# liamliaw/medical-image-segmentation-with-visual-prompts

Hardware: NVIDIA B200
Metric: 3D patches/sec fwd+bwd (96^3 SwinUNETR+prompts) at 1/2/4/8 B200; attn TFLOP/s (higher is better)
Workload: dtype bf16

## Files before the change

### include/pwa.h

```cpp
#ifndef PWA_H_
#define PWA_H_

#include <stddef.h>
#include <stdint.h>

#ifdef __cplusplus
extern "C" {
#endif

#define PWA_VERSION 100

enum { PWA_OK = 0, PWA_ERR_ARG = -1, PWA_ERR_UNSUPPORTED = -2, PWA_ERR_CUDA = -3 };
enum { PWA_F32 = 0, PWA_BF16 = 1 };

typedef struct pwa_geom {
  int32_t dims[3];
  int32_t ws[3];
  int32_t shift[3];
  int32_t pads[6];
  int32_t sp[3];
  int32_t nwin[3];
  int32_t data_lo[3];
  int32_t crop_lo[3];
  int32_t P;
  int32_t N;
  int32_t masked;
  int32_t padded;
} pwa_geom;


int pwa_version(void);
const char* pwa_last_error(void);

int pwa_geometry(const int32_t dims[3], const int32_t ws[3], const int32_t shift_cfg[3], pwa_geom* out);

int pwa_region_ids(const pwa_geom* g, uint8_t* ids_host);

int pwa_attn_sel_table(const uint8_t* ids_host, int P, int N, uint32_t* table_host);

int pwa_index_map(const pwa_geom* g, int which, int32_t* map_host);


int pwa_partition(const void* x, void* tokens, int B, int C, const pwa_geom* g, int use_crop_lo,
                  int dtype, void* stream);

int pwa_reverse(const void* tokens, void* x, int B, int C, const pwa_geom* g, int use_crop_lo,
                int dtype, void* stream);

int pwa_reverse_add(const void* tokens_a, const void* tokens_b, void* x, int B, int C, const pwa_geom* g,
                    int use_crop_lo, int dtype, void* stream);

int pwa_gather_rows(const void* src_a, const void* src_b, void* dst, const int32_t* map, int B,
                    int64_t rows_src, int64_t rows_dst, int C, int dtype, void* stream);

int pwa_colsum_f32(const float* src, float* dst, int S, int64_t n, void* stream);

int pwa_colsum_rows(const void* x, float* dst, int64_t rows, int C, int dtype, void* stream);

int pwa_dropout(const void* x, void* y, int64_t n, float p_drop, const void* seed_dev, int dtype, void* stream);

int pwa_dropout_colsum(const void* x, void* y, int64_t rows, int C, float p_drop, const void* seed_dev, float* colsum,
                       int dtype, void* stream);


typedef struct pwa_attn_shape {
  int32_t B, P, C, heads, I;
  int32_t ws[3];
  float scale;
  float p_drop;
  uint64_t seed, offset;
  int32_t ld_qkv;
  int32_t ld_p;
  const void* seed_dev;
  const void* sel_table;
  void* work;
} pwa_attn_shape;

int pwa_attn_fwd(const void* q, const void* k, const void* v, const void* kp, const void* vp,
                 const float* th, const float* tw, const float* td, const float* tok,
                 const uint8_t* ids, void* out, float* lse, const pwa_attn_shape* s, int dtype,
                 int impl, void* stream);


int pwa_attn_bwd(const void* q, const void* k, const void* v, const void* kp, const void* vp,
                 const float* th, const float* tw, const float* td, const float* tok,
                 const uint8_t* ids, const void* out, const float* lse, const void* dout,
                 void* dq, void* dk, void* dv, float* dkp, float* dvp,
                 float* dth, float* dtw, float* dtd, float* dtok, float* delta,
                 const pwa_attn_shape* s, int dtype, int impl, void* stream);


int pwa_bias_tables_fwd(const float* enc_h, const float* enc_w, const float* enc_d, const float* wc_h,
                        const float* wc_w, const float* wc_d, const float* enc_tok, const float* w_tok,
                        float* th, float* tw, float* td, float* tok, int heads, int E, const int32_t ws[3],
                        const int32_t cap[3], int I, void* stream);

int pwa_bias_tables_bwd(const float* enc_h, const float* enc_w, const float* enc_d, const float* wc_h,
                        const float* wc_w, const float* wc_d, const float* enc_tok, const float* w_tok,
                        const float* dth, const float* dtw, const float* dtd, const float* dtok,
                        float* denc_h, float* denc_w, float* denc_d, float* dwc_h, float* dwc_w, float* dwc_d,
                        float* denc_tok, float* dw_tok, int heads, int E, const int32_t ws[3],
                        const int32_t cap[3], int I, void* stream);


int pwa_ln_fwd(const void* x, const void* res, const float* gamma, const float* beta, void* sum_out, void* y,
               float* mean, float* rstd, int64_t rows, int C, float eps, int dtype, void* stream);

int pwa_ln_bwd(const void* dy, const void* x, const float* gamma, const float* mean, const float* rstd,
               const void* dres, void* dx, float* dgamma, float* dbeta, int64_t rows, int C, int dtype, void* stream);

int pwa_ln_bwd2(const void* dy, const void* x, const float* gamma, const float* mean, const float* rstd,
                const void* dres, void* dx, float* dgamma, float* dbeta, float* dres_colsum, float* dx_colsum,
                int64_t rows, int C, int dtype, void* stream);


int pwa_token_gemm_supported(int C, int Cout);
int pwa_token_gemm_fwd(const void* x, const void* res, const float* gamma, const float* beta, const void* W, const void* bias,
                       void* sum_out, void* ln_out, void* y, float* mean, float* rstd, int64_t T, int C, int Cout, float eps,
                       float p_drop, const void* seed_dev, void* stream);

int pwa_attn_tc_supported(const pwa_attn_shape* s, int dtype);

typedef struct pwa_dense_attn {
  int32_t B, P, heads, dh, nq, nk;
  int32_t ld_q, ld_k, ld_v;
  int64_t bias_stride[4];
  int64_t mask_stride[4];
  float scale, p_drop;
  const void* seed_dev;
} pwa_dense_attn;
int pwa_attn_dense_fwd(const void* q, const void* k, const void* v, const float* bias, const float* mask, void* out, float* lse,
                       const pwa_dense_attn* s, int dtype, void* stream);
int pwa_attn_dense_bwd(const void* q, const void* k, const void* v, const float* bias, const float* mask, const void* out,
                       const float* lse, const void* dout, void* dq, void* dk, void* dv, float* dbias, float* delta,
                       const pwa_dense_attn* s, int dtype, void* stream);

#ifdef __cplusplus
}
#endif
#endif
```

### medical-image-segmentation-with-visual-prompts_b200/_lib.py

```python
from __future__ import annotations

import ctypes as C
import os

_HERE = os.path.dirname(os.path.abspath(__file__))
LIB_PATH = os.path.join(_HERE, "libpwa_b200.so")

PWA_F32, PWA_BF16 = 0, 1


class PwaGeom(C.Structure):
    _fields_ = [
        ("dims", C.c_int32 * 3), ("ws", C.c_int32 * 3), ("shift", C.c_int32 * 3), ("pads", C.c_int32 * 6),
        ("sp", C.c_int32 * 3), ("nwin", C.c_int32 * 3), ("data_lo", C.c_int32 * 3), ("crop_lo", C.c_int32 * 3),
        ("P", C.c_int32), ("N", C.c_int32), ("masked", C.c_int32), ("padded", C.c_int32),
    ]


class PwaAttnShape(C.Structure):
    _fields_ = [
        ("B", C.c_int32), ("P", C.c_int32), ("C", C.c_int32), ("heads", C.c_int32), ("I", C.c_int32),
        ("ws", C.c_int32 * 3), ("scale", C.c_float), ("p_drop", C.c_float),
        ("seed", C.c_uint64), ("offset", C.c_uint64), ("ld_qkv", C.c_int32), ("ld_p", C.c_int32),
        ("seed_dev", C.c_void_p), ("sel_table", C.c_void_p), ("work", C.c_void_p),
    ]


class PwaDenseAttn(C.Structure):
    _fields_ = [
        ("B", C.c_int32), ("P", C.c_int32), ("heads", C.c_int32), ("dh", C.c_int32), ("nq", C.c_int32), ("nk", C.c_int32),
        ("ld_q", C.c_int32), ("ld_k", C.c_int32), ("ld_v", C.c_int32),
        ("bias_stride", C.c_int64 * 4), ("mask_stride", C.c_int64 * 4),
        ("scale", C.c_float), ("p_drop", C.c_float), ("seed_dev", C.c_void_p),
    ]


class PwaError(RuntimeError):
    pass


def _load():
    if not os.path.isfile(LIB_PATH):
        raise ImportError(
            f"{LIB_PATH} not found: the CUDA extension is not built. Run "
            "`python -c 'import __graft_entry__ as g; g.build()'` (or `make -C <package>/csrc`). "
            "This package has no CPU or PyTorch fallback.")
    lib = C.CDLL(LIB_PATH)
    vp, i32, f32p, u8p = C.c_void_p, C.c_int32, C.c_void_p, C.c_void_p
    gp, sp = C.POINTER(PwaGeom), C.POINTER(PwaAttnShape)
    lib.pwa_version.restype = i32
    lib.pwa_last_error.restype = C.c_char_p
    lib.pwa_geometry.argtypes = [C.POINTER(i32), C.POINTER(i32), C.POINTER(i32), gp]
    lib.pwa_region_ids.argtypes = [gp, vp]
    lib.pwa_index_map.argtypes = [gp, i32, vp]
    lib.pwa_attn_sel_table.argtypes = [vp, i32, i32, vp]
    lib.pwa_attn_sel_table.restype = i32
    lib.pwa_partition.argtypes = [vp, vp, i32, i32, gp, i32, i32, vp]
    lib.pwa_reverse.argtypes = [vp, vp, i32, i32, gp, i32, i32, vp]
    lib.pwa_reverse_add.argtypes = [vp, vp, vp, i32, i32, gp, i32, i32, vp]
    lib.pwa_reverse_add.restype = i32
    lib.pwa_gather_rows.argtypes = [vp, vp, vp, vp, i32, C.c_int64, C.c_int64, i32, i32, vp]
    lib.pwa_gather_rows.restype = i32
    lib.pwa_colsum_f32.argtypes = [f32p, f32p, i32, C.c_int64, vp]
    lib.pwa_colsum_f32.restype = i32
    lib.pwa_colsum_rows.argtypes = [vp, f32p, C.c_int64, i32, i32, vp]
    lib.pwa_colsum_rows.restype = i32
    lib.pwa_dropout.argtypes = [vp, vp, C.c_int64, C.c_float, vp, i32, vp]
    lib.pwa_dropout.restype = i32
    lib.pwa_dropout_colsum.argtypes = [vp, vp, C.c_int64, i32, C.c_float, vp, vp, i32, vp]
    lib.pwa_dropout_colsum.restype = i32
    lib.pwa_token_gemm_supported.argtypes = [i32, i32]
    lib.pwa_token_gemm_supported.restype = i32
    lib.pwa_token_gemm_fwd.argtypes = [vp] * 11 + [C.c_int64, i32, i32, C.c_float, C.c_float, vp, vp]
    lib.pwa_token_gemm_fwd.restype = i32
    if hasattr(lib, "pwa_debug_fwd_timeline"):
        lib.pwa_debug_fwd_timeline.argtypes = [vp, i32]
        lib.pwa_debug_fwd_timeline.restype = i32
    lib.pwa_attn_tc_supported.argtypes = [sp, i32]
    dp = C.POINTER(PwaDenseAttn)
    lib.pwa_attn_dense_fwd.argtypes = [vp] * 7 + [dp, i32, vp]
    lib.pwa_attn_dense_bwd.argtypes = [vp] * 13 + [dp, i32, vp]
    lib.pwa_attn_dense_fwd.restype = lib.pwa_attn_dense_bwd.restype = i32
    lib.pwa_attn_fwd.argtypes = [vp] * 5 + [f32p] * 4 + [u8p, vp, f32p, sp, i32, i32, vp]
    lib.pwa_attn_bwd.argtypes = [vp] * 5 + [f32p] * 4 + [u8p, vp, f32p, vp] + [vp] * 3 + [f32p] * 7 + [sp, i32, i32, vp]
    i64, f32 = C.c_int64, C.c_float
    lib.pwa_ln_fwd.argtypes = [vp, vp, f32p, f32p, vp, vp, f32p, f32p, i64, i32, f32, i32, vp]
    lib.pwa_ln_bwd.argtypes = [vp, vp, f32p, f32p, f32p, vp, vp, f32p, f32p, i64, i32, i32, vp]
    lib.pwa_ln_bwd2.argtypes = [vp, vp, f32p, f32p, f32p, vp, vp, f32p, f32p, f32p, f32p, i64, i32, i32, vp]
    lib.pwa_ln_fwd.restype = lib.pwa_ln_bwd.restype = lib.pwa_ln_bwd2.restype = i32
    i32p = C.POINTER(i32)
    lib.pwa_bias_tables_fwd.argtypes = [f32p] * 8 + [f32p] * 4 + [i32, i32, i32p, i32p, i32, vp]
    lib.pwa_bias_tables_bwd.argtypes = [f32p] * 8 + [f32p] * 4 + [f32p] * 8 + [i32, i32, i32p, i32p, i32, vp]
    lib.pwa_bias_tables_fwd.restype = lib.pwa_bias_tables_bwd.restype = i32
    for name in ("pwa_geometry", "pwa_region_ids", "pwa_index_map", "pwa_partition", "pwa_reverse",
                 "pwa_attn_tc_supported", "pwa_attn_fwd", "pwa_attn_bwd"):
        getattr(lib, name).restype = i32
    return lib


lib = _load()

EXPORTED_SYMBOLS = ("pwa_version", "pwa_last_error", "pwa_geometry", "pwa_region_ids", "pwa_index_map", "pwa_attn_sel_table",
                    "pwa_partition", "pwa_reverse", "pwa_reverse_add", "pwa_gather_rows", "pwa_colsum_f32", "pwa_colsum_rows", "pwa_dropout", "pwa_dropout_colsum", "pwa_token_gemm_supported", "pwa_token_gemm_fwd", "pwa_attn_fwd", "pwa_attn_bwd", "pwa_attn_tc_supported", "pwa_attn_dense_fwd", "pwa_attn_dense_bwd",
                    "pwa_ln_fwd", "pwa_ln_bwd", "pwa_ln_bwd2", "pwa_bias_tables_fwd", "pwa_bias_tables_bwd")


def check(rc: int, what: str):
    if rc != 0:
        msg = lib.pwa_last_error().decode("utf-8", "replace")
        if rc == -1 and "not compatible with the number of heads" in msg:
            raise ValueError(msg)
        if rc == -2:
            raise NotImplementedError(f"{what}: {msg}")
        raise PwaError(f"{what} failed (rc={rc}): {msg}")
```

### medical-image-segmentation-with-visual-prompts_b200/functional.py

```python
from __future__ import annotations

import ctypes as C
from typing import Optional, Sequence

import functools

import torch

from . import _lib
from .geometry import Geometry

_DT = {torch.float32: _lib.PWA_F32, torch.bfloat16: _lib.PWA_BF16}


class KernelStats:
    enabled = False
    timing = False
    launches = 0
    records = []

    @classmethod
    def reset(cls, enabled=True, timing=False):
        cls.enabled, cls.timing, cls.launches, cls.records = enabled, timing, 0, []

    @classmethod
    def summary(cls):
        out = {}
        for name, e0, e1, work in cls.records:
            c, ms, w = out.get(name, (0, 0.0, 0.0))
            out[name] = (c + 1, ms + e0.elapsed_time(e1), w + work)
        return out


class _timed:
    def __init__(self, name, n_kernels, work, t):
        self.name, self.n, self.work, self.t = name, n_kernels, work, t

    def __enter__(self):
        if KernelStats.enabled:
            KernelStats.launches += self.n
            if KernelStats.timing:
                self.e0 = torch.cuda.Event(enable_timing=True)
                self.e1 = torch.cuda.Event(enable_timing=True)
                self.e0.record(torch.cuda.current_stream(self.t.device))
        return self

    def __exit__(self, *exc):
        if KernelStats.enabled and KernelStats.timing:
            self.e1.record(torch.cuda.current_stream(self.t.device))
            KernelStats.records.append((self.name, self.e0, self.e1, self.work))
        return False


def _dtype_code(t: torch.Tensor) -> int:
    if t.dtype not in _DT:
        raise TypeError(f"pwa kernels support float32 and bfloat16, got {t.dtype}")
    return _DT[t.dtype]


def _require_cuda(*ts):
    for t in ts:
        if t is not None and not t.is_cuda:
            raise RuntimeError("pwa_b200 has no CPU path: tensors must live on a CUDA device (sm_100a)")


def _stream(t: torch.Tensor):
    return C.c_void_p(torch.cuda.current_stream(t.device).cuda_stream)


def _ptr(t: Optional[torch.Tensor]):
    return C.c_void_p(0 if t is None else t.data_ptr())


def _force_bits(force_generic, force_word, force_vec):
    return (2 if force_generic else 0) | (4 if force_word else 0) | (8 if force_vec else 0)


def _partition_raw(x: torch.Tensor, geom: Geometry, crop_lo: int, force_generic: bool = False,
                   force_word: bool = False, force_vec: bool = False) -> torch.Tensor:
    B, Cc = x.shape[:2]
    out = torch.empty((B, geom.P, geom.N, Cc), dtype=x.dtype, device=x.device)
    with torch.cuda.device(x.device), _timed("partition", 1, 2.0 * out.numel() * out.element_size(), x):
        rc = _lib.lib.pwa_partition(_ptr(x), _ptr(out), B, Cc, geom.ref(), crop_lo | _force_bits(force_generic, force_word, force_vec),
                                    _dtype_code(x), _stream(x))
    _lib.check(rc, "pwa_partition")
    return out


def _reverse_raw(tok: torch.Tensor, geom: Geometry, crop_lo: int, force_generic: bool = False,
                 force_word: bool = False, force_vec: bool = False) -> torch.Tensor:
    B, _, _, Cc = tok.shape
    out = torch.empty((B, Cc, *geom.dims), dtype=tok.dtype, device=tok.device)
    with torch.cuda.device(tok.device), _timed("reverse", 1, 2.0 * tok.numel() * tok.element_size(), tok):
        rc = _lib.lib.pwa_reverse(_ptr(tok), _ptr(out), B, Cc, geom.ref(), crop_lo | _force_bits(force_generic, force_word, force_vec),
                                  _dtype_code(tok), _stream(tok))
    _lib.check(rc, "pwa_reverse")
    return out


class _Partition(torch.autograd.Function):
    @staticmethod
    def forward(ctx, x, geom):
        ctx.geom = geom
        return _partition_raw(x.contiguous(), geom, 0)

    @staticmethod
    def backward(ctx, g):
        return _reverse_raw(g.contiguous(), ctx.geom, 0), None


class _Reverse(torch.autograd.Function):
    @staticmethod
    def forward(ctx, tok, geom):
        ctx.geom = geom
        return _reverse_raw(tok.contiguous(), geom, 1)

    @staticmethod
    def backward(ctx, g):
        return _partition_raw(g.contiguous(), ctx.geom, 1), None


class _ReverseAdd(torch.autograd.Function):
    @staticmethod
    def forward(ctx, tok_a, tok_b, geom):
        ctx.geom = geom
        tok_a, tok_b = tok_a.contiguous(), tok_b.contiguous()
        B, _, _, Cc = tok_a.shape
        out = torch.empty((B, Cc, *geom.dims), dtype=tok_a.dtype, device=tok_a.device)
        with torch.cuda.device(tok_a.device), _timed("reverse", 1, 3.0 * tok_a.numel() * tok_a.element_size(), tok_a):
            rc = _lib.lib.pwa_reverse_add(_ptr(tok_a), _ptr(tok_b), _ptr(out), B, Cc, geom.ref(), 1, _dtype_code(tok_a),
                                          _stream(tok_a))
        _lib.check(rc, "pwa_reverse_add")
        return out

    @staticmethod
    def backward(ctx, g):
        d = _partition_raw(g.contiguous(), ctx.geom, 1)
        return d, d, None


def reverse_add_tokens(tok_a: torch.Tensor, tok_b: torch.Tensor, geom: Geometry) -> torch.Tensor:
    _require_cuda(tok_a, tok_b)
    if tok_a.shape != tok_b.shape or tok_a.dtype != tok_b.dtype or tuple(tok_a.shape[1:3]) != (geom.P, geom.N):
        raise ValueError("reverse_add_tokens: mismatching token tensors")
    return _ReverseAdd.apply(tok_a, tok_b, geom)


def partition_tokens(x: torch.Tensor, geom: Geometry) -> torch.Tensor:
    _require_cuda(x)
    if tuple(x.shape[2:]) != geom.dims:
        raise ValueError(f"feature map {tuple(x.shape[2:])} does not match geometry {geom.dims}")
    return _Partition.apply(x, geom)


def reverse_tokens(tok: torch.Tensor, geom: Geometry) -> torch.Tensor:
    _require_cuda(tok)
    if tuple(tok.shape[1:3]) != (geom.P, geom.N):
        raise ValueError(f"token tensor {tuple(tok.shape)} does not match geometry P={geom.P} N={geom.N}")
# ... 511 lines not shown
        return dx, None, None, (None if db is None else db.to(ctx.bias_dtype))


def dropout_colsum_supported(C: int) -> bool:
    return C % 4 == 0 and C <= 1024


def seeded_dropout(x: torch.Tensor, p_drop: float, seed: Optional[torch.Tensor] = None, bias_of_x=None) -> torch.Tensor:
    _require_cuda(x, seed)
    if p_drop <= 0.0:
        return x
    if seed is None:
        seed = new_dropout_seed(x.device)
    if seed.dtype != torch.int32 or seed.numel() < 2:
        raise ValueError("seeded_dropout: seed must be an int32 tensor with two words")
    return _SeededDropout.apply(x, float(p_drop), seed, bias_of_x)


def prompted_window_attention_packed(qkv, kvp, th, tw, td, tok, ids, heads: int, ws: Sequence[int], scale: float,
                                     impl: int = IMPL_AUTO, p_drop: float = 0.0, seed: Optional[torch.Tensor] = None) -> torch.Tensor:
    _require_cuda(qkv, kvp, th, tw, td, tok, ids)
    if qkv.shape[-1] % (3 * heads) != 0:
        raise ValueError('WindowAttention: The dimension is not compatible with the number of heads!')
    if qkv.dim() != 4:
        raise ValueError(f"prompted_window_attention_packed: qkv must be [B,P,N,3C], got {tuple(qkv.shape)}")
    _check_attn_side_inputs(qkv.shape[0], qkv.shape[1], qkv.shape[2], qkv.shape[3] // 3, qkv.dtype, kvp, None, 2, th, tw, td, tok,
                            ids, heads, ws)
    if p_drop > 0 and seed is None:
        seed = new_dropout_seed(qkv.device)
    return _WindowAttentionPacked.apply(qkv, kvp, th, tw, td, tok, ids, heads, tuple(ws), scale, impl, float(p_drop), seed)


def _mm_f32(a, b):
    if a.dtype == torch.float32:
        return torch.mm(a, b)
    try:
        return torch.mm(a, b, out_dtype=torch.float32)
    except (TypeError, RuntimeError):
        return torch.mm(a, b).float()


@functools.lru_cache(maxsize=None)
def _token_split(T):
    cands = [d for d in range(32, 161) if T % d == 0]
    return min(cands, key=lambda d: abs(d - 72)) if cands else 0


def colsum_f32(part):
    _require_cuda(part)
    part = part.contiguous()
    out = torch.empty(part.shape[1:], dtype=torch.float32, device=part.device)
    with torch.cuda.device(part.device), _timed("colsum", 1, 4.0 * part.numel(), part):
        rc = _lib.lib.pwa_colsum_f32(_ptr(part), _ptr(out), part.shape[0], out.numel(), _stream(part))
    _lib.check(rc, "pwa_colsum_f32")
    return out


def colsum_rows(x2):
    _require_cuda(x2)
    T, Cc = x2.shape
    e = 16 // x2.element_size()
    if x2.dtype not in (torch.float32, torch.bfloat16) or not x2.is_contiguous() or Cc % e or Cc // e > 512 or x2.data_ptr() % 16:
        return x2.sum(dim=0, dtype=torch.float32)
    if T == 0:
        return torch.zeros(Cc, dtype=torch.float32, device=x2.device)
    out = torch.empty(Cc, dtype=torch.float32, device=x2.device)
    with torch.cuda.device(x2.device), _timed("colsum_rows", 1, float(x2.numel() * x2.element_size()), x2):
        rc = _lib.lib.pwa_colsum_rows(_ptr(x2), _ptr(out), T, Cc, _dtype_code(x2), _stream(x2))
    _lib.check(rc, "pwa_colsum_rows")
    return out


def _wgrad(dy2, x2):
    T, co = dy2.shape
    ci = x2.shape[1]
    if dy2.dtype != torch.float32 and dy2.is_contiguous() and x2.is_contiguous():
        S = 0
        if T >= 16384 and co * ci <= 40960:
            S = _token_split(T)
        elif T >= 8192 and T % 8 == 0 and co * ci <= 131072:
            S = 8
        if S:
            try:
                part = torch.bmm(dy2.view(S, T // S, co).transpose(1, 2), x2.view(S, T // S, ci), out_dtype=torch.float32)
            except (TypeError, RuntimeError):
                part = None
            if part is not None:
                return colsum_f32(part)
    return _mm_f32(dy2.t(), x2)


class _MultiLinear(torch.autograd.Function):

    @staticmethod
    def forward(ctx, x, bias, lowp, bias_grad, lowp_bias, *weights):
        w = lowp if lowp is not None else (weights[0] if len(weights) == 1 else torch.cat(weights, dim=0)).detach().to(x.dtype)
        x2 = x.reshape(-1, x.shape[-1])
        if bias is not None:
            y = torch.addmm(lowp_bias if lowp_bias is not None else bias.detach().to(x.dtype), x2, w.t())
        else:
            y = torch.mm(x2, w.t())
        ctx.save_for_backward(x2, w)
        ctx.meta = (x.shape, [wt.shape[0] for wt in weights], [wt.dtype for wt in weights],
                    None if (bias is None or not bias_grad) else bias.dtype)
        return y.reshape(*x.shape[:-1], w.shape[0])

    @staticmethod
    def backward(ctx, dy):
        x2, w = ctx.saved_tensors
        xshape, rows, wdts, bdt = ctx.meta
        dy2 = dy.reshape(-1, dy.shape[-1])
        dx = torch.mm(dy2, w).reshape(xshape) if ctx.needs_input_grad[0] else None
        db = colsum_rows(dy2).to(bdt) if bdt is not None and ctx.needs_input_grad[1] else None
        dws = [None] * len(rows)
        if any(ctx.needs_input_grad[5:]):
            dw = _wgrad(dy2, x2)
            o = 0
            for i, r in enumerate(rows):
                if ctx.needs_input_grad[5 + i]:
                    dws[i] = dw[o:o + r].to(wdts[i])
                o += r
        return (dx, db, None, None, None, *dws)


def multi_linear(x, bias, *weights, lowp=None, bias_grad=True, lowp_bias=None):
    return _MultiLinear.apply(x, bias, lowp, bias_grad, lowp_bias, *weights)


def token_gemm_supported(C: int, Cout: int, dtype) -> bool:
    return dtype == torch.bfloat16 and bool(_lib.lib.pwa_token_gemm_supported(int(C), int(Cout)))


def token_gemm_profitable(C: int, rows: int) -> bool:
    return C <= 48 and rows >= 32768


def _token_gemm_raw(x2, res2, g32, b32, w, bias, want_sum, want_ln, want_stats, eps, p_drop, seed):
    rows, Cc = x2.shape
    Cout = w.shape[0]
    dev = x2.device
    y = torch.empty((rows, Cout), dtype=x2.dtype, device=dev)
    s = torch.empty_like(x2) if want_sum else None
    z = torch.empty_like(x2) if want_ln else None
    mean = torch.empty(rows, dtype=torch.float32, device=dev) if want_stats else None
    rstd = torch.empty(rows, dtype=torch.float32, device=dev) if want_stats else None
    nbytes = ((1 if res2 is None else 2) + (1 if want_sum else 0) + (1 if want_ln else 0)) * x2.numel() * 2 + y.numel() * 2
    with torch.cuda.device(dev), _timed("token_gemm", 1, float(nbytes), x2):
        rc = _lib.lib.pwa_token_gemm_fwd(_ptr(x2), _ptr(res2), _ptr(g32), _ptr(b32), _ptr(w), _ptr(bias), _ptr(s), _ptr(z), _ptr(y),
                                         _ptr(mean), _ptr(rstd), rows, Cc, Cout, float(eps), float(p_drop), _ptr(seed), _stream(x2))
    _lib.check(rc, "pwa_token_gemm_fwd")
    return y, s, z, mean, rstd


def _ln_backward_raw(dy, x, g32, mean, rstd, dres, want_res_colsum, want_x_colsum):
    Cc = x.shape[-1]
    rows = x.numel() // Cc
    dx = torch.empty_like(x)
    f32 = dict(dtype=torch.float32, device=x.device)
    dg, db = torch.empty(Cc, **f32), torch.empty(Cc, **f32)
    dbr = torch.empty(Cc, **f32) if want_res_colsum and dres is not None else None
    dbx = torch.empty(Cc, **f32) if want_x_colsum else None
    nbytes = (3 if dres is None else 4) * x.numel() * x.element_size()
    with torch.cuda.device(x.device), _timed("ln_bwd", 1, float(nbytes), x):
        rc = _lib.lib.pwa_ln_bwd2(_ptr(dy), _ptr(x), _ptr(g32), _ptr(mean), _ptr(rstd), _ptr(dres), _ptr(dx), _ptr(dg), _ptr(db),
                                  _ptr(dbr), _ptr(dbx), rows, Cc, _dtype_code(x), _stream(x))
    _lib.check(rc, "pwa_ln_bwd")
    return dx, dg, db, dbr, dbx


class _LnLinearPass(torch.autograd.Function):

    @staticmethod
    def forward(ctx, x, gamma, beta, eps, lowp_w, *weights):
        x = x.contiguous()
        Cc = x.shape[-1]
        g32, b32 = gamma.detach().float().contiguous(), beta.detach().float().contiguous()
        w = lowp_w if lowp_w is not None else (weights[0] if len(weights) == 1 else torch.cat(weights, dim=0)).detach().to(x.dtype)
        w = w.contiguous()
        y, _, tokens, mean, rstd = _token_gemm_raw(x.view(-1, Cc), None, g32, b32, w, None, False, True, True, eps, 0.0, None)
        ctx.save_for_backward(x, g32, mean, rstd, tokens, w)
        ctx.meta = ([wt.shape[0] for wt in weights], [wt.dtype for wt in weights], (gamma.dtype, beta.dtype))
        return x.view_as(x), y.view(*x.shape[:-1], w.shape[0])

    @staticmethod
    def backward(ctx, dalias, dy):
        x, g32, mean, rstd, tokens, w = ctx.saved_tensors
        rows_w, wdts, (gd, bd) = ctx.meta
        dy2 = dy.reshape(-1, dy.shape[-1])
        dtok = torch.mm(dy2, w)
        dws = [None] * len(rows_w)
        if any(ctx.needs_input_grad[5:]):
            dw = _wgrad(dy2.contiguous(), tokens)
            o = 0
            for i, r in enumerate(rows_w):
                if ctx.needs_input_grad[5 + i]:
                    dws[i] = dw[o:o + r].to(wdts[i])
                o += r
        dres = dalias.contiguous().view(-1, x.shape[-1]) if dalias is not None else None
        dx, dg, db, _, _ = _ln_backward_raw(dtok, x.view(-1, x.shape[-1]), g32, mean, rstd, dres, False, False)
        return (dx.view_as(x), dg.to(gd), db.to(bd), None, None, *dws)


def ln_linear_pass(x, gamma, beta, eps, lowp_w, *weights):
    _require_cuda(x, gamma, beta, lowp_w)
    return _LnLinearPass.apply(x, gamma, beta, eps, lowp_w, *weights)


class _DropAddLnLinear(torch.autograd.Function):

    @staticmethod
    def forward(ctx, a, res, gamma, beta, eps, lowp_w, lowp_b, p_drop, seed, weight, bias, bias_of_a):
        a, res = a.contiguous(), res.contiguous()
        Cc = a.shape[-1]
        g32, b32 = gamma.detach().float().contiguous(), beta.detach().float().contiguous()
        w = (lowp_w if lowp_w is not None else weight.detach().to(a.dtype)).contiguous()
        bb = (lowp_b if lowp_b is not None else bias.detach().to(a.dtype)).contiguous() if bias is not None else None
        m, s, z, mean, rstd = _token_gemm_raw(a.view(-1, Cc), res.view(-1, Cc), g32, b32, w, bb, True, True, True, eps, p_drop, seed)
        ctx.save_for_backward(s, g32, mean, rstd, z, w, seed)
        ctx.meta = (float(p_drop), weight.dtype, None if bias is None else bias.dtype, None if bias_of_a is None else bias_of_a.dtype,
                    (gamma.dtype, beta.dtype), a.shape)
        return s.view_as(a), m.view(*a.shape[:-1], w.shape[0])

    @staticmethod
    def backward(ctx, ds, dm):
        s, g32, mean, rstd, z, w, seed = ctx.saved_tensors
        p_drop, wdt, bdt, badt, (gd, bd), ashape = ctx.meta
        Cc = s.shape[-1]
        dm2 = dm.reshape(-1, dm.shape[-1]).contiguous()
        dz = torch.mm(dm2, w)
        dw = _wgrad(dm2, z).to(wdt) if ctx.needs_input_grad[9] else None
        ds2 = ds.contiguous().view(-1, Cc) if ds is not None else None
        want_b = bdt is not None and ctx.needs_input_grad[10] and ds2 is not None
        want_ba = badt is not None and ctx.needs_input_grad[11]
        dx, dg, db, dbr, dbx = _ln_backward_raw(dz, s, g32, mean, rstd, ds2, want_b, want_ba and p_drop == 0.0)
        dbias = dbr.to(bdt) if dbr is not None else (colsum_rows(dm2).to(bdt) if bdt is not None and ctx.needs_input_grad[10] else None)
        if p_drop > 0.0:
            da = torch.empty_like(dx)
            dba = None
            with torch.cuda.device(dx.device), _timed("dropout", 1, 2.0 * dx.numel() * dx.element_size(), dx):
                if want_ba and dropout_colsum_supported(Cc):
                    dba = torch.empty(Cc, dtype=torch.float32, device=dx.device)
                    rc = _lib.lib.pwa_dropout_colsum(_ptr(dx), _ptr(da), dx.numel() // Cc, Cc, p_drop, _ptr(seed), _ptr(dba),
                                                     _dtype_code(dx), _stream(dx))
                else:
                    rc = _lib.lib.pwa_dropout(_ptr(dx), _ptr(da), dx.numel(), p_drop, _ptr(seed), _dtype_code(dx), _stream(dx))
            _lib.check(rc, "pwa_dropout")
            if want_ba and dba is None:
                dba = colsum_rows(da)
        else:
            da, dba = dx, dbx
        return (da.view(ashape), dx.view(ashape), dg.to(gd), db.to(bd), None, None, None, None, None, dw, dbias,
                None if dba is None else dba.to(badt))


def drop_add_ln_linear(a, res, gamma, beta, eps, lowp_w, lowp_b, p_drop, seed, weight, bias, bias_of_a=None):
    _require_cuda(a, res, gamma, beta, weight, seed)
    if a.shape != res.shape or a.dtype != res.dtype:
        raise ValueError("drop_add_ln_linear: a and res must match")
    if p_drop > 0 and seed is None:
        seed = new_dropout_seed(a.device)
    return _DropAddLnLinear.apply(a, res, gamma, beta, eps, lowp_w, lowp_b, float(p_drop), seed, weight, bias, bias_of_a)
```

Baseline: 786.0.

## Fuse LayerNorm-linear backward into one tcgen05 kernel with wgrad and recompute

Adds a fused backward kernel for the LN+linear token GEMM. It computes dZ = dY·W on tensor cores into TMEM, accumulates the weight gradient per CTA, and does the LayerNorm backward in registers. It recomputes the normalized activations from x instead of saving them in forward, which cuts memory traffic and removes several separate launches (mm, wgrad, ln_bwd, colsum). Per-CTA partial sums are reduced afterwards with colsum_f32, which adds a reduction step and restricts the path to bf16 with small C.

Measured after the change: 794.8, median of 6. 1.01x the previous value.

```diff
diff --git a/include/pwa.h b/include/pwa.h
--- a/include/pwa.h
+++ b/include/pwa.h
@@ -119,6 +119,11 @@
                        void* sum_out, void* ln_out, void* y, float* mean, float* rstd, int64_t T, int C, int Cout, float eps,
                        float p_drop, const void* seed_dev, void* stream);
 
+int pwa_token_gemm_bwd_supported(int C, int Cout);
+int64_t pwa_token_gemm_bwd_ctas(int64_t T);
+int pwa_token_gemm_bwd(const void* dy, const void* x, const void* dres, const float* mean, const float* rstd, const float* gamma,
+                       const float* beta, const void* W, void* dx, float* part, int64_t T, int C, int Cout, void* stream);
+
 int pwa_attn_tc_supported(const pwa_attn_shape* s, int dtype);
 
 typedef struct pwa_dense_attn {
diff --git a/medical-image-segmentation-with-visual-prompts_b200/_lib.py b/medical-image-segmentation-with-visual-prompts_b200/_lib.py
--- a/medical-image-segmentation-with-visual-prompts_b200/_lib.py
+++ b/medical-image-segmentation-with-visual-prompts_b200/_lib.py
@@ -73,6 +73,12 @@
     lib.pwa_token_gemm_supported.restype = i32
     lib.pwa_token_gemm_fwd.argtypes = [vp] * 11 + [C.c_int64, i32, i32, C.c_float, C.c_float, vp, vp]
     lib.pwa_token_gemm_fwd.restype = i32
+    lib.pwa_token_gemm_bwd_supported.argtypes = [i32, i32]
+    lib.pwa_token_gemm_bwd_supported.restype = i32
+    lib.pwa_token_gemm_bwd_ctas.argtypes = [C.c_int64]
+    lib.pwa_token_gemm_bwd_ctas.restype = C.c_int64
+    lib.pwa_token_gemm_bwd.argtypes = [vp] * 10 + [C.c_int64, i32, i32, vp]
+    lib.pwa_token_gemm_bwd.restype = i32
     if hasattr(lib, "pwa_debug_fwd_timeline"):
         lib.pwa_debug_fwd_timeline.argtypes = [vp, i32]
         lib.pwa_debug_fwd_timeline.restype = i32
@@ -101,7 +107,7 @@
 lib = _load()
 
 EXPORTED_SYMBOLS = ("pwa_version", "pwa_last_error", "pwa_geometry", "pwa_region_ids", "pwa_index_map", "pwa_attn_sel_table",
-                    "pwa_partition", "pwa_reverse", "pwa_reverse_add", "pwa_gather_rows", "pwa_colsum_f32", "pwa_colsum_rows", "pwa_dropout", "pwa_dropout_colsum", "pwa_token_gemm_supported", "pwa_token_gemm_fwd", "pwa_attn_fwd", "pwa_attn_bwd", "pwa_attn_tc_supported", "pwa_attn_dense_fwd", "pwa_attn_dense_bwd",
+                    "pwa_partition", "pwa_reverse", "pwa_reverse_add", "pwa_gather_rows", "pwa_colsum_f32", "pwa_colsum_rows", "pwa_dropout", "pwa_dropout_colsum", "pwa_token_gemm_supported", "pwa_token_gemm_fwd", "pwa_token_gemm_bwd_supported", "pwa_token_gemm_bwd_ctas", "pwa_token_gemm_bwd", "pwa_attn_fwd", "pwa_attn_bwd", "pwa_attn_tc_supported", "pwa_attn_dense_fwd", "pwa_attn_dense_bwd",
                     "pwa_ln_fwd", "pwa_ln_bwd", "pwa_ln_bwd2", "pwa_bias_tables_fwd", "pwa_bias_tables_bwd")
 
 
diff --git a/medical-image-segmentation-with-visual-prompts_b200/csrc/token_gemm_bwd.cu b/medical-image-segmentation-with-visual-prompts_b200/csrc/token_gemm_bwd.cu
--- /dev/null
+++ b/medical-image-segmentation-with-visual-prompts_b200/csrc/token_gemm_bwd.cu
@@ -0,0 +1,332 @@
+#include "common.cuh"
+#include "tc_common.cuh"
+
+namespace pwa {
+using namespace tc;
+
+namespace {
+
+constexpr int kTM = 128;
+constexpr int kChunk = kTM * 16;
+constexpr uint32_t kColW = 64;
+constexpr uint32_t kTmemCols = 256;
+
+struct TokBwdParams {
+  const __nv_bfloat16 *dy, *x, *dres, *W;
+  const float *mean, *rstd, *gamma, *beta;
+  __nv_bfloat16* dx;
+  float* part;
+  long T;
+  int Cout;
+};
+
+struct BwdSmem {
+  uint32_t z, one, dy, x, r, w, total;
+};
+__host__ __device__ inline BwdSmem bwd_layout(int C, int Cout) {
+  BwdSmem s;
+  uint32_t o = 0;
+  s.z = o; o += C / 8 * kChunk;
+  s.one = o; o += kChunk;
+  s.dy = o; o += Cout / 8 * kChunk;
+  s.x = o; o += C / 8 * kChunk;
+  s.r = o; o += C / 8 * kChunk;
+  s.w = o; o += Cout / 8 * C * 16;
+  if (o < s.z + 16 * kChunk) o = s.z + 16 * kChunk;
+  s.total = o < 96 * 1024 ? 96 * 1024 : o;
+  return s;
+}
+
+__device__ __forceinline__ void cp_async16(void* dst_smem, const void* src, uint32_t src_bytes) {
+  asm volatile("cp.async.cg.shared.global [%0], [%1], 16, %2;" ::"r"(smem_u32(dst_smem)), "l"(src), "r"(src_bytes) : "memory");
+}
+__device__ __forceinline__ void cp_async_commit() { asm volatile("cp.async.commit_group;" ::: "memory"); }
+__device__ __forceinline__ void cp_async_wait_all() { asm volatile("cp.async.wait_group 0;" ::: "memory"); }
+__device__ __forceinline__ void bulk_s2g(void* dst_gmem, const void* src_smem, uint32_t bytes) {
+  asm volatile("cp.async.bulk.global.shared::cta.bulk_group [%0], [%1], %2;" ::"l"(dst_gmem), "r"(smem_u32(src_smem)), "r"(bytes)
+               : "memory");
+}
+__device__ __forceinline__ void bulk_commit() { asm volatile("cp.async.bulk.commit_group;" ::: "memory"); }
+__device__ __forceinline__ void bulk_wait_read_all() { asm volatile("cp.async.bulk.wait_group.read 0;" ::: "memory"); }
+__device__ __forceinline__ void unpack8(const uint4& w, float (&v)[8]) {
+  const uint32_t u[4] = {w.x, w.y, w.z, w.w};
+#pragma unroll
+  for (int i = 0; i < 4; ++i) {
+    v[2 * i] = __uint_as_float(u[i] << 16);
+    v[2 * i + 1] = __uint_as_float(u[i] & 0xffff0000u);
+  }
+}
+__device__ __forceinline__ uint4 pack8(const float (&v)[8]) {
+  return make_uint4(pack_bf16(v[0], v[1]), pack_bf16(v[2], v[3]), pack_bf16(v[4], v[5]), pack_bf16(v[6], v[7]));
+}
+
+__device__ __forceinline__ void load_canonical(uint8_t* dst, const __nv_bfloat16* src, long row0, int rows, int width, int tid) {
+  const int n8 = width / 8;
+  for (int i = tid; i < kTM * n8; i += kTM) {
+    const int c = 2 * (i / (2 * kTM)) + (i & 1), r = (i >> 1) & (kTM - 1);
+    const bool ok = r < rows;
+    cp_async16(dst + c * kChunk + r * 16, src + (ok ? (row0 + r) * width + c * 8 : 0), ok ? 16u : 0u);
+  }
+}
+
+template <int C>
+__global__ void __launch_bounds__(kTM, 2) token_gemm_bwd_ln_kernel(TokBwdParams p) {
+  constexpr int NC8 = C / 8;
+  extern __shared__ __align__(128) uint8_t smem[];
+  __shared__ __align__(8) uint64_t bar_mma;
+  __shared__ uint32_t tmem_base_s;
+  __shared__ __align__(16) float gam_s[C], bet_s[C];
+  const int tid = threadIdx.x, warp = tid >> 5;
+  const int Cout = p.Cout, NJ8 = Cout / 8;
+  const bool wgrad = p.part != nullptr;
+  const BwdSmem L = bwd_layout(C, Cout);
+  uint8_t* Zs = smem + L.z;
+  uint8_t* Ds = smem + L.dy;
+  *reinterpret_cast<uint4*>(smem + L.one + tid * 16) = make_uint4(0x3f803f80u, 0x3f803f80u, 0x3f803f80u, 0x3f803f80u);
+  uint8_t* Xs = smem + L.x;
+  uint8_t* Rs = smem + L.r;
+  uint8_t* Ws = smem + L.w;
+  const long n_tiles = (p.T + kTM - 1) / kTM;
+  long tile = blockIdx.x;
+
+  for (int i = tid; i < Cout * C / 8; i += kTM) cp_async16(Ds + i * 16, p.W + (size_t)i * 8, 16u);
+  cp_async_commit();
+  cp_async_wait_all();
+  __syncthreads();
+  {
+    const __nv_bfloat16* Wst = reinterpret_cast<const __nv_bfloat16*>(Ds);
+    for (int i = tid; i < NJ8 * C; i += kTM) {
+      const int jc = i / C, n = i - jc * C;
+      float v[8];
+#pragma unroll
+      for (int e = 0; e < 8; ++e) v[e] = __bfloat162float(Wst[(jc * 8 + e) * C + n]);
+      *reinterpret_cast<uint4*>(Ws + (jc * C + n) * 16) = pack8(v);
+    }
+  }
+  __syncthreads();
+  if (tile < n_tiles) {
+    const int rows = (int)min((long)kTM, p.T - tile * kTM);
+    load_canonical(Ds, p.dy, tile * kTM, rows, Cout, tid);
+    load_canonical(Xs, p.x, tile * kTM, rows, C, tid);
+    if (p.dres) load_canonical(Rs, p.dres, tile * kTM, rows, C, tid);
+    cp_async_commit();
+  }
+  for (int i = tid; i < C; i += kTM) {
+    gam_s[i] = p.gamma[i];
+    bet_s[i] = p.beta[i];
+  }
+  if (tid == 0) {
+    mbar_init(&bar_mma, 1);
+    fence_mbar_init();
+  }
+  if (warp == 0) tmem_alloc(&tmem_base_s, kTmemCols);
+  fence_proxy_async_smem();
+  tc_fence_before();
+  __syncthreads();
+  tc_fence_after();
+  const uint32_t tmem = tmem_base_s;
+  const uint32_t trow = tmem + ((uint32_t)(warp * 32) << 16);
+  const uint32_t idesc_dg = make_idesc_bf16(128, C, 0, 0);
+  const uint32_t idesc_wg = make_idesc_bf16(128, Cout, 1, 1);
+  const float invC = 1.f / (float)C;
+  float ag[C], ab[C];
+#pragma unroll
+  for (int c = 0; c < C; ++c) ag[c] = ab[c] = 0.f;
+  uint32_t phase = 0;
+  bool first = true;
+
+  for (; tile < n_tiles; tile += gridDim.x) {
+    const long row0 = tile * kTM;
+    const int rows = (int)min((long)kTM, p.T - row0);
+    const long row = row0 + tid;
+    const bool live = tid < rows;
+    const float mean = live ? __ldg(p.mean + row) : 0.f, rstd = live ? __ldg(p.rstd + row) : 0.f;
+    cp_async_wait_all();
+    fence_proxy_async_smem();
+    if (tid == 0) bulk_wait_read_all();
+    __syncthreads();
+    uint4 xr[NC8], rr[NC8];
+#pragma unroll
+    for (int c = 0; c < NC8; ++c) {
+      xr[c] = *reinterpret_cast<const uint4*>(Xs + c * kChunk + tid * 16);
+      rr[c] = p.dres ? *reinterpret_cast<const uint4*>(Rs + c * kChunk + tid * 16) : make_uint4(0, 0, 0, 0);
+      uint4 w = make_uint4(0, 0, 0, 0);
+      if (live) {
+        float v[8];
+        unpack8(xr[c], v);
+#pragma unroll
+        for (int e = 0; e < 8; ++e) v[e] = fmaf((v[e] - mean) * rstd, gam_s[c * 8 + e], bet_s[c * 8 + e]);
+        w = pack8(v);
+      }
+      *reinterpret_cast<uint4*>(Zs + c * kChunk + tid * 16) = w;
+    }
+    fence_proxy_async_smem();
+    tc_fence_before();
+    __syncthreads();
+    tc_fence_after();
+    const long next = tile + gridDim.x;
+    const int next_rows = next < n_tiles ? (int)min((long)kTM, p.T - next * kTM) : 0;
+    if (next < n_tiles) {
+      load_canonical(Xs, p.x, next * kTM, next_rows, C, tid);
+      if (p.dres) load_canonical(Rs, p.dres, next * kTM, next_rows, C, tid);
+    }
+    if (warp == 0) {
+      if (elect_one_sync()) {
+        for (int ks = 0; ks < Cout / 16; ++ks) {
+          const uint64_t da = make_smem_desc(smem_u32(Ds) + ks * 2 * kChunk, kChunk, 128);
+          const uint64_t db = make_smem_desc(smem_u32(Ws) + ks * 2 * (C * 16), C * 16, 128);
+          mma_ss(tmem, da, db, idesc_dg, ks > 0);
+        }
+        if (wgrad) {
+          for (int kk = 0; kk < kTM / 16; ++kk) {
+            const uint64_t da = make_smem_desc(smem_u32(Zs) + kk * 256, 128, kChunk);
+            const uint64_t db = make_smem_desc(smem_u32(Ds) + kk * 256, 128, kChunk);
+            mma_ss(tmem + kColW, da, db, idesc_wg, (!first) | (kk > 0));
+          }
+        }
+        mma_commit(&bar_mma);
+      }
+      __syncwarp();
+    }
+    mbar_wait(&bar_mma, phase);
+    tc_fence_after();
+    phase ^= 1;
+    first = false;
+    if (next < n_tiles) load_canonical(Ds, p.dy, next * kTM, next_rows, Cout, tid);
+    cp_async_commit();
+    float d[C];
+#pragma unroll
+    for (int c = 0; c < C / 16; ++c) {
+      uint32_t r[16];
+      tmem_ld16(trow + c * 16, r);
+      tmem_wait_ld();
+#pragma unroll
+      for (int e = 0; e < 16; ++e) d[c * 16 + e] = __uint_as_float(r[e]);
+    }
+    tc_fence_before();
+    if (live) {
+      float s1 = 0.f, s2 = 0.f;
+#pragma unroll
+      for (int c = 0; c < NC8; ++c) {
+        float v[8];
+        unpack8(xr[c], v);
+#pragma unroll
+        for (int e = 0; e < 8; ++e) {
+          const int k = c * 8 + e;
+          const float xh = (v[e] - mean) * rstd;
+          const float g = d[k] * gam_s[k];
+          s1 += g;
+          s2 = fmaf(g, xh, s2);
+          ag[k] = fmaf(d[k], xh, ag[k]);
+          ab[k] += d[k];
+        }
+      }
+      s1 *= invC;
+      s2 *= invC;
+#pragma unroll
+      for (int c = 0; c < NC8; ++c) {
+        float v[8], rs[8];
+        unpack8(xr[c], v);
+        unpack8(rr[c], rs);
+#pragma unroll
+        for (int e = 0; e < 8; ++e) {
+          const int k = c * 8 + e;
+          const float xh = (v[e] - mean) * rstd;
+          v[e] = rstd * (d[k] * gam_s[k] - s1 - xh * s2) + rs[e];
+        }
+        *reinterpret_cast<uint4*>(Zs + (size_t)tid * C * 2 + c * 16) = pack8(v);
+      }
+    }
+    fence_proxy_async_smem();
+    __syncthreads();
+    if (tid == 0) {
+      bulk_s2g(p.dx + row0 * C, Zs, (uint32_t)rows * C * 2);
+      bulk_commit();
+    }
+  }
+  cp_async_wait_all();
+  if (tid == 0) bulk_wait_read_all();
+  __syncthreads();
+
+  if (wgrad) {
+    float* out = p.part + (size_t)blockIdx.x * ((size_t)Cout * C + 2 * C + Cout);
+    if (first) {
+      for (int i = tid; i < Cout * C + 2 * C + Cout; i += kTM) out[i] = 0.f;
+    } else {
+      if (warp * 32 <= C) {
+        for (int j = 0; j < Cout; j += 16) {
+          uint32_t r[16];
+          tmem_ld16(trow + kColW + j, r);
+          tmem_wait_ld();
+          if (tid < C) {
+#pragma unroll
+            for (int e = 0; e < 16; ++e) out[(size_t)(j + e) * C + tid] = __uint_as_float(r[e]);
+          } else if (tid == C) {
+#pragma unroll
+            for (int e = 0; e < 16; ++e) out[(size_t)Cout * C + 2 * C + j + e] = __uint_as_float(r[e]);
+          }
+        }
+      }
+      constexpr int RS = 2 * C + 1;
+      float* red = reinterpret_cast<float*>(smem);
+#pragma unroll
+      for (int c = 0; c < C; ++c) {
+        red[tid * RS + c] = ag[c];
+        red[tid * RS + C + c] = ab[c];
+      }
+      __syncthreads();
+      for (int c = tid; c < 2 * C; c += kTM) {
+        float s = 0.f;
+        for (int t = 0; t < kTM; ++t) s += red[t * RS + c];
+        out[(size_t)Cout * C + c] = s;
+      }
+    }
+  }
+  tc_fence_before();
+  __syncthreads();
+  if (warp == 0) tmem_dealloc(tmem, kTmemCols);
+}
+
+long bwd_grid(long T) {
+  const long n_tiles = (T + kTM - 1) / kTM;
+  long grid = 148L * 2;
+  return grid > n_tiles ? (n_tiles < 1 ? 1 : n_tiles) : grid;
+}
+
+}
+
+}
+
+using namespace pwa;
+
+extern "C" int pwa_token_gemm_bwd_supported(int C, int Cout) {
+  return (C % 16 == 0 && C >= 16 && C <= 48 && (Cout == C || Cout == 3 * C)) ? 1 : 0;
+}
+
+extern "C" int64_t pwa_token_gemm_bwd_ctas(int64_t T) { return bwd_grid((long)T); }
+
+extern "C" int pwa_token_gemm_bwd(const void* dy, const void* x, const void* dres, const float* mean, const float* rstd,
+                                  const float* gamma, const float* beta, const void* W, void* dx, float* part, int64_t T, int C,
+                                  int Cout, void* stream) {
+  PWA_CHECK_ARG(dy && x && mean && rstd && gamma && beta && W && dx, "pwa_token_gemm_bwd: null pointer");
+  PWA_CHECK_ARG(pwa_token_gemm_bwd_supported(C, Cout), "pwa_token_gemm_bwd: need C %% 16 == 0, 16 <= C <= 48, Cout = C or 3C (C=%d Cout=%d)",
+                C, Cout);
+  PWA_CHECK_ARG(T >= 0, "pwa_token_gemm_bwd: T=%lld", (long long)T);
+  if (T == 0) return PWA_OK;
+  TokBwdParams p = {};
+  p.dy = (const __nv_bfloat16*)dy; p.x = (const __nv_bfloat16*)x; p.dres = (const __nv_bfloat16*)dres; p.W = (const __nv_bfloat16*)W;
+  p.mean = mean; p.rstd = rstd; p.gamma = gamma; p.beta = beta;
+  p.dx = (__nv_bfloat16*)dx; p.part = part;
+  p.T = T; p.Cout = Cout;
+  const BwdSmem L = bwd_layout(C, Cout);
+  void (*kern)(TokBwdParams) = nullptr;
+  switch (C) {
+    case 16: kern = token_gemm_bwd_ln_kernel<16>; break;
+    case 32: kern = token_gemm_bwd_ln_kernel<32>; break;
+    default: kern = token_gemm_bwd_ln_kernel<48>; break;
+  }
+  PWA_CUDA_OK(cudaFuncSetAttribute(kern, cudaFuncAttributeMaxDynamicSharedMemorySize, (int)L.total));
+  kern<<<(unsigned)bwd_grid((long)T), kTM, L.total, (cudaStream_t)stream>>>(p);
+  PWA_CUDA_OK(cudaGetLastError());
+  return PWA_OK;
+}
diff --git a/medical-image-segmentation-with-visual-prompts_b200/functional.py b/medical-image-segmentation-with-visual-prompts_b200/functional.py
--- a/medical-image-segmentation-with-visual-prompts_b200/functional.py
+++ b/medical-image-segmentation-with-visual-prompts_b200/functional.py
@@ -4,6 +4,7 @@
 from typing import Optional, Sequence
 
 import functools
+import os
 
 import torch
 
@@ -821,6 +822,34 @@
     return y, s, z, mean, rstd
 
 
+_NO_TOKEN_BWD = os.environ.get("PWA_NO_TOKEN_BWD", "0") == "1"
+
+
+def token_gemm_bwd_supported(C: int, Cout: int, dtype) -> bool:
+    return dtype == torch.bfloat16 and not _NO_TOKEN_BWD and bool(_lib.lib.pwa_token_gemm_bwd_supported(int(C), int(Cout)))
+
+
+def _token_gemm_bwd_raw(dy2, x2, dres2, mean, rstd, g32, b32, w, want_param_grads):
+    rows, Cc = x2.shape
+    Cout = w.shape[0]
+    dx = torch.empty_like(x2)
+    part = None
+    if want_param_grads:
+        part = torch.empty((int(_lib.lib.pwa_token_gemm_bwd_ctas(rows)), Cout * Cc + 2 * Cc + Cout), dtype=torch.float32, device=x2.device)
+        if rows == 0:
+            part.zero_()
+    nbytes = (dy2.numel() + (2 if dres2 is None else 3) * x2.numel()) * 2
+    with torch.cuda.device(x2.device), _timed("token_gemm_bwd", 1, float(nbytes), x2):
+        rc = _lib.lib.pwa_token_gemm_bwd(_ptr(dy2), _ptr(x2), _ptr(dres2), _ptr(mean), _ptr(rstd), _ptr(g32), _ptr(b32), _ptr(w),
+                                         _ptr(dx), _ptr(part), rows, Cc, Cout, _stream(x2))
+    _lib.check(rc, "pwa_token_gemm_bwd")
+    if part is None:
+        return dx, None, None, None, None
+    tot = colsum_f32(part)
+    n = Cout * Cc
+    return dx, tot[:n].view(Cout, Cc), tot[n:n + Cc], tot[n + Cc:n + 2 * Cc], tot[n + 2 * Cc:]
+
+
 def _ln_backward_raw(dy, x, g32, mean, rstd, dres, want_res_colsum, want_x_colsum):
     Cc = x.shape[-1]
     rows = x.numel() // Cc
@@ -846,16 +875,30 @@
         g32, b32 = gamma.detach().float().contiguous(), beta.detach().float().contiguous()
         w = lowp_w if lowp_w is not None else (weights[0] if len(weights) == 1 else torch.cat(weights, dim=0)).detach().to(x.dtype)
         w = w.contiguous()
-        y, _, tokens, mean, rstd = _token_gemm_raw(x.view(-1, Cc), None, g32, b32, w, None, False, True, True, eps, 0.0, None)
-        ctx.save_for_backward(x, g32, mean, rstd, tokens, w)
-        ctx.meta = ([wt.shape[0] for wt in weights], [wt.dtype for wt in weights], (gamma.dtype, beta.dtype))
+        fused_bwd = token_gemm_bwd_supported(Cc, w.shape[0], x.dtype)
+        y, _, tokens, mean, rstd = _token_gemm_raw(x.view(-1, Cc), None, g32, b32, w, None, False, not fused_bwd, True, eps, 0.0,
+                                                   None)
+        ctx.save_for_backward(x, g32, b32, mean, rstd, tokens, w)
+        ctx.meta = ([wt.shape[0] for wt in weights], [wt.dtype for wt in weights], (gamma.dtype, beta.dtype), fused_bwd)
         return x.view_as(x), y.view(*x.shape[:-1], w.shape[0])
 
     @staticmethod
     def backward(ctx, dalias, dy):
-        x, g32, mean, rstd, tokens, w = ctx.saved_tensors
-        rows_w, wdts, (gd, bd) = ctx.meta
+        x, g32, b32, mean, rstd, tokens, w = ctx.saved_tensors
+        rows_w, wdts, (gd, bd), fused_bwd = ctx.meta
         dy2 = dy.reshape(-1, dy.shape[-1])
+        if fused_bwd:
+            dres = dalias.contiguous().view(-1, x.shape[-1]) if dalias is not None else None
+            want = any(ctx.needs_input_grad[1:3]) or any(ctx.needs_input_grad[5:])
+            dx, dw, dg, db, _ = _token_gemm_bwd_raw(dy2.contiguous(), x.view(-1, x.shape[-1]), dres, mean, rstd, g32, b32, w, want)
+            dws = [None] * len(rows_w)
+            o = 0
+            for i, r in enumerate(rows_w):
+                if ctx.needs_input_grad[5 + i]:
+                    dws[i] = dw[o:o + r].to(wdts[i])
+                o += r
+            return (dx.view_as(x), dg.to(gd) if ctx.needs_input_grad[1] else None, db.to(bd) if ctx.needs_input_grad[2] else None,
+                    None, None, *dws)
         dtok = torch.mm(dy2, w)
         dws = [None] * len(rows_w)
         if any(ctx.needs_input_grad[5:]):
@@ -884,25 +927,34 @@
         g32, b32 = gamma.detach().float().contiguous(), beta.detach().float().contiguous()
         w = (lowp_w if lowp_w is not None else weight.detach().to(a.dtype)).contiguous()
         bb = (lowp_b if lowp_b is not None else bias.detach().to(a.dtype)).contiguous() if bias is not None else None
-        m, s, z, mean, rstd = _token_gemm_raw(a.view(-1, Cc), res.view(-1, Cc), g32, b32, w, bb, True, True, True, eps, p_drop, seed)
-        ctx.save_for_backward(s, g32, mean, rstd, z, w, seed)
+        fused_bwd = token_gemm_bwd_supported(Cc, w.shape[0], a.dtype)
+        m, s, z, mean, rstd = _token_gemm_raw(a.view(-1, Cc), res.view(-1, Cc), g32, b32, w, bb, True, not fused_bwd, True, eps,
+                                              p_drop, seed)
+        ctx.save_for_backward(s, g32, b32, mean, rstd, z, w, seed)
         ctx.meta = (float(p_drop), weight.dtype, None if bias is None else bias.dtype, None if bias_of_a is None else bias_of_a.dtype,
-                    (gamma.dtype, beta.dtype), a.shape)
+                    (gamma.dtype, beta.dtype), a.shape, fused_bwd)
         return s.view_as(a), m.view(*a.shape[:-1], w.shape[0])
 
     @staticmethod
     def backward(ctx, ds, dm):
-        s, g32, mean, rstd, z, w, seed = ctx.saved_tensors
-        p_drop, wdt, bdt, badt, (gd, bd), ashape = ctx.meta
+        s, g32, b32, mean, rstd, z, w, seed = ctx.saved_tensors
+        p_drop, wdt, bdt, badt, (gd, bd), ashape, fused_bwd = ctx.meta
         Cc = s.shape[-1]
         dm2 = dm.reshape(-1, dm.shape[-1]).contiguous()
-        dz = torch.mm(dm2, w)
-        dw = _wgrad(dm2, z).to(wdt) if ctx.needs_input_grad[9] else None
         ds2 = ds.contiguous().view(-1, Cc) if ds is not None else None
-        want_b = bdt is not None and ctx.needs_input_grad[10] and ds2 is not None
         want_ba = badt is not None and ctx.needs_input_grad[11]
-        dx, dg, db, dbr, dbx = _ln_backward_raw(dz, s, g32, mean, rstd, ds2, want_b, want_ba and p_drop == 0.0)
-        dbias = dbr.to(bdt) if dbr is not None else (colsum_rows(dm2).to(bdt) if bdt is not None and ctx.needs_input_grad[10] else None)
+        if fused_bwd:
+            want = any(ctx.needs_input_grad[i] for i in (2, 3, 9, 10))
+            dx, dw, dg, db, dbias = _token_gemm_bwd_raw(dm2, s, ds2, mean, rstd, g32, b32, w, want)
+            dw = dw.to(wdt) if ctx.needs_input_grad[9] else None
+            dbias = dbias.to(bdt) if bdt is not None and ctx.needs_input_grad[10] else None
+            dbx = colsum_rows(dx) if want_ba and p_drop == 0.0 else None
+        else:
+            dz = torch.mm(dm2, w)
+            dw = _wgrad(dm2, z).to(wdt) if ctx.needs_input_grad[9] else None
+            want_b = bdt is not None and ctx.needs_input_grad[10] and ds2 is not None
+            dx, dg, db, dbr, dbx = _ln_backward_raw(dz, s, g32, mean, rstd, ds2, want_b, want_ba and p_drop == 0.0)
+            dbias = dbr.to(bdt) if dbr is not None else (colsum_rows(dm2).to(bdt) if bdt is not None and ctx.needs_input_grad[10] else None)
         if p_drop > 0.0:
             da = torch.empty_like(dx)
             dba = None
@@ -918,7 +970,8 @@
                 dba = colsum_rows(da)
         else:
             da, dba = dx, dbx
-        return (da.view(ashape), dx.view(ashape), dg.to(gd), db.to(bd), None, None, None, None, None, dw, dbias,
+        return (da.view(ashape), dx.view(ashape), None if dg is None else dg.to(gd), None if db is None else db.to(bd), None, None,
+                None, None, None, dw, dbias,
                 None if dba is None else dba.to(badt))
 
 
```
